# tjcunhao/dpo

Hardware: NVIDIA H100
Metric: rtr_iters_per_sec_sphere2500 (higher is better)
Workload: dtype f64

## Files before the change

dpo_b200/csrc/dpgo_capi.cu:

```cuda
#include <cuda_runtime.h>
#include <algorithm>
#include <chrono>
#include <cmath>
#include <cstdio>
#include <cstdlib>
#include <cstring>
#include <memory>
#include <numeric>
#include <string>
#include <vector>

#include "dpgo_devbuf.cuh"
#include "dpgo_kernels.cuh"

using dpgo::DevBuf;

namespace {

thread_local std::string g_last_error;

int fail(int code, const std::string &msg) {
  g_last_error = msg;
  return code;
}
// ... 275 lines not shown
    DPGO_CUDA(dpgo::launch_pack_sym(D.pinv.get(), (int)N, nchunks, D.sym_segptr.get(), nseg, D.sym_off.get(), D.ppack.get(),
                                    p->stream));
    DPGO_CUDA(cudaStreamSynchronize(p->stream));
    D.sym_ok = 1;
  }
  return DPGO_OK;
}

void nd_fill_info(const dpgo::nd::Hierarchy &H, const dpgo::nd::Plan &P, int64_t *info) {
  for (int i = 0; i < 16; ++i) info[i] = 0;
  int smax = 0, bmax = 0;
  for (const auto &m : H.nodes) { smax = std::max(smax, (int)m.own.size() * H.dh); bmax = std::max(bmax, (int)m.bnd.size() * H.dh); }
  info[0] = H.nstages; info[1] = (int64_t)H.nodes.size(); info[2] = (int64_t)P.phases.size(); info[3] = H.blob_doubles * 8;
  info[4] = P.bytes_per_apply; info[5] = smax; info[6] = bmax; info[7] = H.nd_depth; info[8] = (int64_t)P.steps.size();
  info[9] = (int64_t)P.jobs.size(); info[10] = (int64_t)P.epis.size(); info[11] = P.max_ytiles; info[12] = P.max_slots;
}

dpgo::nd::Options nd_options(int grid, int r, bool cluster = false) {
  dpgo::nd::Options opt;
  opt.grid = grid;
  opt.r = r;
  if (cluster) opt.t_phase_us = 2.0;
  opt.warps = dpgo::OPT_THREADS / 32;
  opt.ycap_tiles = dpgo::ND_YCAP_TILES;
  opt.slot_cap = dpgo::ND_SLOT_CAP;
  if (const char *e = std::getenv("DPGO_ND_CUTS")) opt.force_ncuts = std::atoi(e);
  if (const char *e = std::getenv("DPGO_ND_LEAF")) opt.leaf_size = std::max(1, std::atoi(e));
  if (const char *e = std::getenv("DPGO_ND_TPHASE_US")) opt.t_phase_us = std::atof(e);
  if (const char *e = std::getenv("DPGO_ND_BW_GBS")) opt.bw_gbs = std::atof(e);
  if (const char *e = std::getenv("DPGO_ND_TTILE_US")) opt.t_tile_us = std::atof(e);
// ... 14 lines not shown
  nd::Plan plan;
  std::vector<double> blob;
  auto H = std::make_unique<nd::Hierarchy>();
  try {
    const nd::Options opt = nd_options(p->grid, p->r, p->cluster);
    nd::BsrView Q{p->n, p->dh, p->bsr.h_rowptr.data(), p->bsr.h_bcol.data(), p->bsr.h_bval.data()};
    nd::build_hierarchy(Q, opt, *H);
    nd::build_numeric(Q, opt, *H, blob);
    nd::build_plan(*H, opt, plan);
  } catch (const std::exception &e) {
    return fail(DPGO_ERR_UNSUPPORTED, std::string("sparse exact preconditioner setup: ") + e.what());
  }
  if (plan.max_ytiles > dpgo::ND_YCAP_TILES || plan.max_slots > dpgo::ND_SLOT_CAP)
    return fail(DPGO_ERR_UNSUPPORTED, "sparse exact preconditioner: plan exceeds the shared-memory capacities");
  dpgo_problem::Nd &F = p->nd;
  nd_fill_info(*H, plan, F.info);
  if ((int)plan.phases.size() > dpgo::nd::MAX_PHASES)
    return fail(DPGO_ERR_UNSUPPORTED, "sparse exact preconditioner: too many phases");
  F.H = std::move(H);
  dpgo::KNd &K = F.k;
  for (size_t k = 0; k < plan.phases.size(); ++k) { K.dir[k] = plan.phases[k].dir; K.cta0[k] = plan.phases[k].cta0; }
  K.max_ytiles = std::max(plan.max_ytiles, 1);
  K.max_slots = std::max(plan.max_slots, 1);
  K.max_gathers = K.max_ytiles;
  DPGO_CUDA(F.cta_phase.assign(plan.cta_phase.data(), plan.cta_phase.size(), p->stream));
  DPGO_CUDA(F.steps.assign(plan.steps.data(), plan.steps.size(), p->stream));
  DPGO_CUDA(F.gathers.assign(plan.gathers.data(), plan.gathers.size(), p->stream));
  DPGO_CUDA(F.jobs.assign(plan.jobs.data(), plan.jobs.size(), p->stream));
  DPGO_CUDA(F.epis.assign(plan.epis.data(), plan.epis.size(), p->stream));
  DPGO_CUDA(F.csrc.assign(plan.csrc.data(), plan.csrc.size(), p->stream));
  DPGO_CUDA(F.blob.assign(blob.data(), blob.size(), p->stream));
  K.cta_phase = F.cta_phase.get(); K.steps = F.steps.get(); K.gathers = F.gathers.get(); K.jobs = F.jobs.get();
  K.epis = F.epis.get(); K.csrc = F.csrc.get(); K.blob = F.blob.get();
  const size_t tile = (size_t)p->ts;
  DPGO_CUDA(F.TX.alloc(tile * (size_t)p->n));
  DPGO_CUDA(F.C.alloc(tile * (size_t)F.H->cbuf_tiles));
  K.TX = F.TX.get();
  K.C = F.C.get();
  DPGO_CUDA(cudaMemsetAsync(K.TX, 0, sizeof(double) * tile * (size_t)p->n, p->stream));
// ... 748 lines not shown
  namespace nd = dpgo::nd;
  try {
    nd::Options opt = nd_options(grid, r);
    opt.force_ncuts = force_cuts;
    opt.shift = shift;
    if (leaf_size > 0) opt.leaf_size = leaf_size;
    nd::BsrView Q{n, dh, rowptr.data(), bc.data(), bv.data()};
    nd::Hierarchy H;
    nd::Plan plan;
    std::vector<double> blob;
    nd::build_hierarchy(Q, opt, H);
    nd::build_numeric(Q, opt, H, blob);
    nd::build_plan(H, opt, plan);
    if (plan.max_ytiles > opt.ycap_tiles || plan.max_slots > opt.slot_cap)
      return fail(DPGO_ERR_UNSUPPORTED, "plan exceeds the shared-memory capacities");
    nd::emulate_apply(H, plan, blob, r, V_host, Z_host);
    if (info16) nd_fill_info(H, plan, info16);
    if (const char *dump = std::getenv("DPGO_ND_DUMP_PLAN")) {
      if (FILE *fp = std::fopen(dump, "w")) {
        std::fprintf(fp, "phase,dir,stage,cta,steps,gather_tiles,jobs,job_cols,max_warp_cols,epis\n");
        for (size_t ph = 0; ph < plan.phases.size(); ++ph)
          for (int c = 0; c < plan.grid; ++c) {
            const nd::CtaPhase &cp = plan.cta_phase[(size_t)plan.phases[ph].cta0 + c];
            long gt = 0, nj = 0, jc = 0, ne = 0, mw = 0;
            for (int si = cp.s0; si < cp.s1; ++si) {
              const nd::Step &st = plan.steps[(size_t)si];
              gt += st.g1 - st.g0; nj += st.j1 - st.j0; ne += st.e1 - st.e0;
              std::vector<long> w((size_t)opt.warps, 0);
              for (int j = st.j0; j < st.j1; ++j) { jc += plan.jobs[(size_t)j].ncols; w[(size_t)((j - st.j0) % opt.warps)] += plan.jobs[(size_t)j].ncols + 40; }
              mw += *std::max_element(w.begin(), w.end());
            }
            std::fprintf(fp, "%zu,%d,%d,%d,%d,%ld,%ld,%ld,%ld,%ld\n", ph, plan.phases[ph].dir, plan.phases[ph].stage, c, cp.s1 - cp.s0, gt, nj, jc, mw, ne);
          }
        std::fclose(fp);
      }
    }
  } catch (const std::exception &e) {
    return fail(DPGO_ERR_UNSUPPORTED, std::string("sparse exact preconditioner: ") + e.what());
  }
  return DPGO_OK;
}

static int reassemble_Q(dpgo_problem *p) {
  const dpgo_problem::Edges &E = p->edges;
  DPGO_CUDA(dpgo::launch_assemble_Q(p->bsr.nb, E.cptr.get(), E.contrib.get(), E.T.get(), E.om.get(), E.w.get(), E.sblk.get(),
                                    p->bsr.bval.get(), p->stream));
  DPGO_CUDA(cudaMemcpyAsync(p->bsr.h_bval.data(), p->bsr.bval.get(), sizeof(double) * 16 * (size_t)p->bsr.nb,
// ... 1008 lines not shown
```

dpo_b200/csrc/dpgo_kernels.cu:

```cuda
#include "dpgo_device.cuh"
#include "dpgo_kernels.cuh"
#include "dpgo_rotation.cuh"
#include <cooperative_groups.h>
#include <algorithm>

namespace dpgo {

struct BlockCtx {
  double *sm_warp;
  double *sm_out;
  unsigned epoch;
  int parity;
};

template <int NUSED = NRED>
__device__ __forceinline__ void phase_end(const KParams &kp, BlockCtx &bc, double (&acc)[NRED]) {
  const int lane = threadIdx.x & 31, warp = threadIdx.x >> 5, nwarps = blockDim.x >> 5;
#pragma unroll
  for (int q = 0; q < NUSED; ++q) {
    double v = warp_sum(acc[q]);
    if (lane == 0) bc.sm_warp[warp * NRED + q] = v;
  }
  __syncthreads();
  bc.epoch += gridDim.x;
// ... 598 lines not shown
      }
      double ya[3], sym[3];
      const double z = tangent_project_elem<R, DH>(x, t, it.a, it.c, ya, sym);
      if (ld) {
        Zout[idx] = z;
        acc[0] = fma(z, __ldcg(V + idx), acc[0]);
      }
    }
  }
}

__device__ __forceinline__ int4 ld_int4(const void *p) { return __ldg(reinterpret_cast<const int4 *>(p)); }

template <int R, int DH, bool CLOCK>
__device__ void phase_nd(const KParams &kp, int ph, const double *V, int cb, double *Zout, double *ys, double *slots,
                         int4 *grec, double (&acc)[NRED]) {
  constexpr int TS = R * DH;
  constexpr int SG = SubGroup<R>::SG;
  constexpr int SGW = 32 / SG;
  constexpr int SLOT = nd::PANEL_ROWS * R;
  constexpr int NC = nd::INLINE_CONTRIB;
  const KNd &N = kp.nd;
  const int dir = N.dir[ph];
  const int4 ca = ld_int4(N.cta_phase + N.cta0[ph] + blockIdx.x),
             cbq = ld_int4(reinterpret_cast<const int4 *>(N.cta_phase + N.cta0[ph] + blockIdx.x) + 1);
  const int s0 = ca.x, s1 = ca.y;
  const int lane = threadIdx.x & 31, warp = threadIdx.x >> 5, nwarps = blockDim.x >> 5;
  const int sgw = lane / SG, l = lane & (SG - 1), a = l >> 2, c = l & 3;
  const bool valid = (a < R) && (c < DH);
  const int e = c * R + a;
  const int nsub = nwarps * SGW;
// ... 43 lines not shown
      }
    }
    __syncthreads();
    if (ticking) asm volatile("mov.u64 %0, %%globaltimer;" : "=l"(tg1));
    {
      const int r8 = lane >> 2, k4 = lane & 3;
      const bool bval_lane = (r8 < R);
      int ji = j0 + warp;
      int4 ja = make_int4(0, 0, 0, 0), jb = make_int4(0, 0, 0, 0);
      if (ji < j1) { ja = ld_int4(N.jobs + ji); jb = ld_int4(reinterpret_cast<const int4 *>(N.jobs + ji) + 1); }
      while (ji < j1) {
        const int jn = ji + nwarps;
        int4 na = make_int4(0, 0, 0, 0), nb = make_int4(0, 0, 0, 0);
        if (jn < j1) { na = ld_int4(N.jobs + jn); nb = ld_int4(reinterpret_cast<const int4 *>(N.jobs + jn) + 1); }
        const long long mat = ((long long)(unsigned)ja.x) | ((long long)ja.y << 32);
        const int ncols = ja.z, ycol = ja.w, slot = jb.x, accum = jb.y;
        const double *mp = N.blob + mat + (size_t)k4 * nd::PANEL_ROWS + r8;
        const double *yp = ys + (size_t)(ycol + k4) * R + (bval_lane ? r8 : 0);
        double d0 = 0.0, d1 = 0.0, f0 = 0.0, f1 = 0.0;
        for (int j = 0; j < ncols; j += 32) {
          double am[8], bm[8];
          if (j + 32 <= ncols) {
#pragma unroll
            for (int u = 0; u < 8; ++u) am[u] = ld_stream(mp + (size_t)(j + 4 * u) * nd::PANEL_ROWS);
#pragma unroll
            for (int u = 0; u < 8; ++u) bm[u] = bval_lane ? yp[(size_t)(j + 4 * u) * R] : 0.0;
          } else {
#pragma unroll
            for (int u = 0; u < 8; ++u) am[u] = (j + 4 * u + k4 < ncols) ? ld_stream(mp + (size_t)(j + 4 * u) * nd::PANEL_ROWS) : 0.0;
#pragma unroll
            for (int u = 0; u < 8; ++u) bm[u] = (bval_lane && j + 4 * u + k4 < ncols) ? yp[(size_t)(j + 4 * u) * R] : 0.0;
          }
#pragma unroll
          for (int u = 0; u < 8; u += 2) {
            dmma884(d0, d1, am[u], bm[u]);
            dmma884(f0, f1, am[u + 1], bm[u + 1]);
          }
        }
        d0 += f0;
        d1 += f1;
        {
          double *sl = slots + (size_t)slot * SLOT + r8 * R + 2 * k4;
          if (2 * k4 < R) sl[0] = accum ? sl[0] + d0 : d0;
          if (2 * k4 + 1 < R) sl[1] = accum ? sl[1] + d1 : d1;
        }
        ji = jn; ja = na; jb = nb;
// ... 186 lines not shown
  bc.parity = 0;
  unsigned long long tick_last = 0;
  const bool ticking = FULL && (kp.phase_ns != nullptr) && blockIdx.x == 0 && threadIdx.x == 0;
  auto tick = [&](int kind) {
    if (ticking) {
      unsigned long long t;
      asm volatile("mov.u64 %0, %%globaltimer;" : "=l"(t));
      if (kind >= 0) kp.phase_ns[kind] += t - tick_last;
      tick_last = t;
    }
  };
  tick(-1);
  const dpgo_opt_params_t prm = kp.prm;
  const int precond = prm.precond;
  const bool exact = (precond == DPGO_PRECOND_DENSE_EXACT) || (precond == DPGO_PRECOND_SPARSE_EXACT);
  double acc[NRED];
  double *nd_ys = sV;
  double *nd_slots = sV + (size_t)kp.nd.max_ytiles * R * DH;
  int4 *nd_grec = reinterpret_cast<int4 *>((reinterpret_cast<uintptr_t>(nd_slots + (size_t)kp.nd.max_slots * nd::PANEL_ROWS * R) + 15) & ~(uintptr_t)15);
  auto apply_exact = [&](const double *Vv, int cbx, double *Zout) {
    if (!FULL || precond == DPGO_PRECOND_SPARSE_EXACT) {
      zero(acc);
      for (int ph = 0; ph < kp.nd.nphases; ++ph) {
        phase_nd<R, DH, FULL>(kp, ph, Vv, cbx, Zout, nd_ys, nd_slots, nd_grec, acc);
        if (ph + 1 < kp.nd.nphases) { phase_end<0>(kp, bc, acc); tick(8 + min(ph, 15)); }
      }
      phase_end<1>(kp, bc, acc);
      tick(8 + min(kp.nd.nphases - 1, 15));
    } else {
      if (dense_sym) phase_dense_sym<R>(kp, Vv, ring, sV, sMeta);
      else if (dense_tma) phase_dense_tma<R>(kp, Vv, sV, ring);
      else phase_dense<R>(kp, Vv, sV);
      zero(acc); phase_end<0>(kp, bc, acc);
      tick(1);
      zero(acc); phase_pz<R, DH>(kp, cr, cbx, Vv, Zout, sV, acc);
      phase_end<1>(kp, bc, acc);
      tick(2);
    }
  };
  dpgo_opt_result_t res;
  res.success = 0; res.tcg_status = DPGO_TCG_NOT_RUN; res.tcg_iterations = 0; res.outer_iterations = 0;
  res.rejections = 0; res.spmv_passes = 0; res.precond_applies = 0; res.reserved0 = 0;
  res.f_init = res.gradnorm_init = res.f_opt = res.gradnorm_opt = res.relative_change = res.elapsed_ms = 0.0;
  res.quad_init = res.lin_init = 0.0;

  int cur = 0;

  if (kp.op == OP_PHASE_BENCH) {
    for (int i = 0; i < prm.tr_max_inner; ++i) { zero(acc); acc[0] = 1.0; phase_end<1>(kp, bc, acc); }
    if (blockIdx.x == 0 && threadIdx.x == 0) { res.f_init = acc[0]; *kp.result = res; *kp.bar_epoch = bc.epoch; }
    return;
  }
  if (kp.op == OP_PRECON) {
    if (exact) {
      apply_exact(kp.v[V_AUX], 0, kp.v[V_Z]);
    } else {
      constexpr int TS = R * DH;
      RowIter<R> it(cr);
      const bool valid = (it.a < R) && (it.c < DH);
// ... 312 lines not shown
    tra = fma(s, s, tra);
  }
  const double r2 = om[0] * rot + om[D] * tra;
  if (resid) resid[e] = r2;
  if (fixed && fixed[e]) return;
  const double r = sqrt(r2);
  double wt = 1.0;
  if (cost == 1) wt = 1.0 / r;
  else if (cost == 2) wt = (r < param) ? 1.0 : param / r;
  else if (cost == 3) wt = (r < param) ? 1.0 : 0.0;
  else if (cost == 4) { const double s = 1.0 + r2; wt = 1.0 / (s * s); }
  else if (cost == 5) wt = gnc_tls_weight(r2, mu, param);
  w[e] = wt;
}

template <int R, int DH> static size_t optimize_smem_doubles(const KParams &kp, bool max_only) {
  const size_t base = (OPT_THREADS / 32) * NRED + 2 * NRED + SP_CACHE_INTS / 2;
  const size_t dense = (size_t)DENSE_PER_MAX * R + (size_t)DENSE_RING_DOUBLES + 2 * DENSE_NST + (size_t)SYM_META_DOUBLES;
  if (max_only || kp.prm.precond == DPGO_PRECOND_DENSE_EXACT) return base + dense;
  if (kp.prm.precond == DPGO_PRECOND_SPARSE_EXACT)
    return base + (size_t)kp.nd.max_ytiles * R * DH + (size_t)(kp.nd.max_slots + 1) * nd::PANEL_ROWS * R + 4 * (size_t)kp.nd.max_gathers + 8;
  return base + 8;
}

template <int R, int DH> static void *optimize_kernel(bool full) {
  return full ? (void *)k_optimize<R, DH, true> : (void *)k_optimize<R, DH, false>;
}

template <int R, int DH> static cudaError_t launch_optimize_t(const KParams &kp_in, cudaStream_t stream) {
  KParams kp = kp_in;
  const bool full = (kp.phase_ns != nullptr) || (kp.prm.precond == DPGO_PRECOND_DENSE_EXACT);
  const void *kern = optimize_kernel<R, DH>(full);
  const size_t smem_max = optimize_smem_doubles<R, DH>(kp, true) * sizeof(double);
  static_assert((size_t)ND_YCAP_TILES * R * DH + (size_t)(ND_SLOT_CAP + 1) * nd::PANEL_ROWS * R + 4 * (size_t)ND_YCAP_TILES + 8 <=
                    (size_t)DENSE_PER_MAX * R + (size_t)DENSE_RING_DOUBLES + 2 * DENSE_NST + (size_t)SYM_META_DOUBLES,
                "the sparse plan's capacities must fit the kernel's maximum shared memory");
  kp.smem_doubles = (int)optimize_smem_doubles<R, DH>(kp, false);
  const size_t smem = (size_t)kp.smem_doubles * sizeof(double);
  static bool attr_set[2][64] = {};
  int dev = 0;
  cudaGetDevice(&dev);
  if (dev < 0 || dev >= 64 || !attr_set[full][dev]) {
    cudaError_t e = cudaFuncSetAttribute(kern, cudaFuncAttributeMaxDynamicSharedMemorySize, (int)smem_max);
    if (e != cudaSuccess) return e;
    if (dev >= 0 && dev < 64) attr_set[full][dev] = true;
  }
  {
    static int last_pct[2][64];
    static bool init = false;
    if (!init) { for (int i = 0; i < 64; ++i) last_pct[0][i] = last_pct[1][i] = -1; init = true; }
    const int pct = std::min(100, (int)((smem + 2048) * 100 / (228 * 1024)) + 1);
    if (dev >= 0 && dev < 64 && last_pct[full][dev] != pct) {
      cudaFuncSetAttribute(kern, cudaFuncAttributePreferredSharedMemoryCarveout, pct);
      last_pct[full][dev] = pct;
    }
  }
  if (kp.cluster) {
    static bool np_set[2][64] = {};
// ... 10 lines not shown
    cudaLaunchAttribute at[1];
    at[0].id = cudaLaunchAttributeClusterDimension;
    at[0].val.clusterDim.x = (unsigned)kp.grid;
    at[0].val.clusterDim.y = 1;
    at[0].val.clusterDim.z = 1;
    cfg.attrs = at;
    cfg.numAttrs = 1;
    void *args[] = {(void *)&kp};
    return cudaLaunchKernelExC(&cfg, kern, args);
  }
  void *args[] = {(void *)&kp};
  return cudaLaunchCooperativeKernel(kern, dim3(kp.grid), dim3(OPT_THREADS), args, smem, stream);
}

template <int R, int DH> static int max_cluster_t(int device) {
  const size_t smem = ((OPT_THREADS / 32) * NRED + 2 * NRED + SP_CACHE_INTS / 2 + (size_t)ND_SMEM_NEED_SMALL) * sizeof(double);
  for (int f = 0; f < 2; ++f) cudaFuncSetAttribute(optimize_kernel<R, DH>(f != 0), cudaFuncAttributeNonPortableClusterSizeAllowed, 1);
  for (int cs : {16, 8}) {
    cudaLaunchConfig_t cfg = {};
    cfg.gridDim = dim3(cs);
    cfg.blockDim = dim3(OPT_THREADS);
    cfg.dynamicSmemBytes = smem;
    cudaLaunchAttribute at[1];
    at[0].id = cudaLaunchAttributeClusterDimension;
    at[0].val.clusterDim.x = (unsigned)cs;
    at[0].val.clusterDim.y = 1;
    at[0].val.clusterDim.z = 1;
    cfg.attrs = at;
    cfg.numAttrs = 1;
    int n0 = 0, n1 = 0;
    if (cudaOccupancyMaxActiveClusters(&n0, optimize_kernel<R, DH>(false), &cfg) == cudaSuccess && n0 >= 1 &&
        cudaOccupancyMaxActiveClusters(&n1, optimize_kernel<R, DH>(true), &cfg) == cudaSuccess && n1 >= 1)
      return cs;
  }
  cudaGetLastError();
  return 0;
}

template <int R, int DH> static int max_grid_t(int device) {
  const size_t smem = ((OPT_THREADS / 32) * NRED + 2 * NRED + SP_CACHE_INTS / 2 + (size_t)DENSE_PER_MAX * R + (size_t)DENSE_RING_DOUBLES + 2 * DENSE_NST + (size_t)SYM_META_DOUBLES) * sizeof(double);
  int per_sm = 1, sms = 0;
  for (int f = 0; f < 2; ++f) {
    const void *kern = optimize_kernel<R, DH>(f != 0);
    cudaFuncSetAttribute(kern, cudaFuncAttributeMaxDynamicSharedMemorySize, (int)smem);
    int ps = 0;
    if (cudaOccupancyMaxActiveBlocksPerMultiprocessor(&ps, kern, OPT_THREADS, smem) != cudaSuccess) return 0;
    per_sm = std::min(per_sm, ps);
  }
  if (cudaDeviceGetAttribute(&sms, cudaDevAttrMultiProcessorCount, device) != cudaSuccess) return 0;
  return per_sm > 0 ? sms : 0;
}

cudaError_t launch_optimize(int r, int dh, const KParams &kp, cudaStream_t stream) {
  cudaError_t e = cudaErrorInvalidValue;
  DPGO_DISPATCH(r, dh, e = (launch_optimize_t<R, DH>(kp, stream)));
  return e;
// ... 135 lines not shown
```

dpo_b200/csrc/dpgo_kernels.cuh:

```cuda
#pragma once
#include <cuda_runtime.h>
#include <stdint.h>
#include "../../include/dpgo_b200.h"
#include "nd_precond.h"

namespace dpgo {

enum VecId {
  V_X0 = 0, V_X1,
  V_EG0, V_EG1,
  V_RG0, V_RG1,
  V_Z00, V_Z01,
  V_ETA, V_RES, V_Z,
  V_D0, V_D1,
  V_HD,
  V_T,
  V_XIN,
  V_AUX,
  V_COUNT
};

enum OpCode {
  OP_OPTIMIZE = 0,
  OP_EVAL = 1,
  OP_RHESS = 2,
  OP_PRECON = 3,
  OP_RETRACT = 4,
  OP_PHASE_BENCH = 9,
};

constexpr int NRED = 4;
constexpr int OPT_THREADS = 512;
constexpr int SPMV_GROUP_BLOCKS = 192;
constexpr int ND_YCAP_TILES = 600;
constexpr int ND_SLOT_CAP = 240;
constexpr int ND_SMEM_NEED_SMALL = 16000;
constexpr int SP_CACHE_INTS = 2048;
constexpr int DENSE_PER_MAX = 512;

struct KNd {
  int nphases;
  int max_ytiles, max_slots;
  int max_gathers;
  int dir[nd::MAX_PHASES];
  int cta0[nd::MAX_PHASES];
  const nd::CtaPhase *cta_phase;
  const nd::Step *steps;
  const nd::Gather *gathers;
  const nd::Job *jobs;
  const nd::Epi *epis;
  const int *csrc;
  const double *blob;
  double *TX;
  double *C;
};

struct KParams {
  int n;
// ... 48 lines not shown
        case 3: { constexpr int R = 3, DH = 3; __VA_ARGS__; } break;     \
        case 5: { constexpr int R = 5, DH = 3; __VA_ARGS__; } break;     \
        default: break;                                                  \
      }                                                                  \
    }                                                                    \
  } while (0)

cudaError_t launch_optimize(int r, int dh, const KParams &kp, cudaStream_t stream);
cudaError_t launch_spmv(int r, int dh, int n, const int *rowptr, const int *bcol, const double *bval,
                        const double *X, const double *G, double *out, cudaStream_t stream);
cudaError_t launch_spmv_tma(int r, int dh, int ngroups, const int2 *groups, const int *rowptr, const int *bcol,
                            const double *bval, const double *X, const double *G, double *out, int sms,
                            cudaStream_t stream);
int spmv_group_blocks();
int optimize_max_grid(int r, int dh, int device);
int optimize_max_cluster(int r, int dh, int device);
cudaError_t launch_stiefel_project(int r, int dh, int n, const double *M, double *out, cudaStream_t stream, double c0 = 1.0,
                                   const double *B = nullptr, double c1 = 0.0, const double *C = nullptr, double c2 = 0.0);
cudaError_t launch_pack_tiles(int ts, int count, const int *pose, const double *X, double *out, cudaStream_t stream,
                              const unsigned char *gate = nullptr);
cudaError_t launch_build_G(int r, int dh, int nposes, const int *pose_ids, const int *pose_ptr, const int *edge_slot,
                           const int *edge_out, const double *edge_T, const double *edge_om, const double *gathered,
                           double *G, cudaStream_t stream, const unsigned char *gate = nullptr);
cudaError_t launch_assemble_Q(int64_t nb, const int *cptr, const int2 *contrib, const double *eT, const double *eom, const double *ew,
                              const double *sblk, double *bval, cudaStream_t stream);
cudaError_t launch_edge_weights(int r, int dh, int64_t m, const int *p1, const int *p2, const double *eT, const double *eom,
                                const int *fixed, const double *X, int cost, double mu, double param, double *w, double *resid,
                                cudaStream_t stream);
cudaError_t launch_pack_sym(const double *pinv, int N, int nchunks, const int *segptr, int nseg, const long long *off, double *ppack,
                            cudaStream_t stream);
// ... 65 lines not shown
```

dpo_b200/csrc/nd_precond.cpp:

```cpp
#include "nd_precond.h"

#include <algorithm>
#include <cmath>
#include <cstdio>
#include <cstring>
#include <functional>
#include <numeric>
#include <sstream>
#include <stdexcept>

namespace dpgo {
namespace nd {

namespace {

struct Graph {
  int n = 0;
  std::vector<int> ptr, adj;
};

Graph make_graph(const BsrView &Q) {
  Graph g;
  g.n = Q.n;
  std::vector<std::vector<int>> nb((size_t)Q.n);
// ... 820 lines not shown
  P.grid = opt.grid;
  P.r = opt.r;
  PhaseBuilder pb(H, opt, P);
  for (int st = 0; st < H.nstages; ++st) {
    pb.dir = 0;
    pb.stage = st;
    pb.build();
  }
  for (int st = H.nstages - 2; st >= 0; --st) {
    pb.dir = 1;
    pb.stage = st;
    pb.build();
  }
}

void emulate_apply(const Hierarchy &H, const Plan &P, const std::vector<double> &blob, int r, const double *V, double *Z) {
  const int dh = H.dh, ts = r * dh;
  std::vector<double> TX((size_t)H.n * ts, 0.0), C((size_t)H.cbuf_tiles * ts, 0.0);
  std::vector<double> ys((size_t)std::max(P.max_ytiles, 1) * ts), slots((size_t)std::max(P.max_slots, 1) * PANEL_ROWS * r);
  for (size_t ph = 0; ph < P.phases.size(); ++ph) {
    const Phase &phs = P.phases[ph];
    for (int c = 0; c < P.grid; ++c) {
      const CtaPhase &cph = P.cta_phase[(size_t)phs.cta0 + c];
      const int s0 = cph.s0, s1 = cph.s1;
      if (s1 > s0) {
        const Step &f = P.steps[(size_t)s0];
        if (f.g0 != cph.g0 || f.g1 != cph.g1 || f.j0 != cph.j0 || f.j1 != cph.j1 || f.e0 != cph.e0 || f.e1 != cph.e1)
          throw std::runtime_error("nd: inline first step disagrees with the step table");
      }
      std::fill(slots.begin(), slots.end(), std::nan(""));
      for (int si = s0; si < s1; ++si) {
// ... 2 lines not shown
        for (int gi = st.g0; gi < st.g1; ++gi) {
          const Gather &g = P.gathers[(size_t)gi];
          for (int e = 0; e < ts; ++e) {
            double v = (phs.dir == 0) ? V[(size_t)g.src * ts + e] : TX[(size_t)g.src * ts + e];
            for (int k = 0; k < g.nc; ++k) {
              const int ct = (k < INLINE_CONTRIB) ? g.ci[k] : P.csrc[(size_t)(g.cext + k - INLINE_CONTRIB)];
              v -= C[(size_t)ct * ts + e];
            }
            ys[(size_t)g.ytile * ts + e] = v;
          }
        }
        for (int ji = st.j0; ji < st.j1; ++ji) {
          const Job &jb = P.jobs[(size_t)ji];
          const double *mat = blob.data() + jb.mat;
          double *sl = slots.data() + (size_t)jb.slot * PANEL_ROWS * r;
          for (int row = 0; row < PANEL_ROWS; ++row)
            for (int a = 0; a < r; ++a) {
              double acc = 0.0;
              for (int j = 0; j < jb.ncols; ++j) acc += mat[(size_t)j * PANEL_ROWS + row] * ys[(size_t)(jb.ycol + j) * r + a];
              if (jb.accum) sl[row * r + a] += acc; else sl[row * r + a] = acc;
            }
        }
        for (int ei = st.e0; ei < st.e1; ++ei) {
          const Epi &ep = P.epis[(size_t)ei];
          for (int cc = 0; cc < dh; ++cc)
            for (int a = 0; a < r; ++a) {
              const int e = cc * r + a, row = ep.half * dh + cc;
              double sum = 0.0;
              for (int k = 0; k < ep.nslots; ++k) sum += slots[(size_t)(ep.slot0 + k) * PANEL_ROWS * r + row * r + a];
              if (ep.kind == EPI_F_OWN) {
                TX[(size_t)ep.out * ts + e] = sum;
              } else if (ep.kind == EPI_F_BND) {
                for (int k = 0; k < ep.nc; ++k) {
                  const int ct = (k < INLINE_CONTRIB) ? ep.ci[k] : P.csrc[(size_t)(ep.cext + k - INLINE_CONTRIB)];
// ... 9 lines not shown
                Z[(size_t)ep.aux * ts + e] = x;
              }
            }
        }
      }
    }
  }
}

std::string describe(const Hierarchy &H, const Plan &P) {
  std::ostringstream os;
  os << "nd: n=" << H.n << " depth=" << H.nd_depth << " cuts=[";
  for (size_t k = 0; k < H.cuts.size(); ++k) os << (k ? "," : "") << H.cuts[k];
  os << "] stages=" << H.nstages << " nodes=" << H.nodes.size() << " blob=" << (H.blob_doubles * 8) / 1e6 << "MB phases=" << P.phases.size()
     << " bytes/apply=" << P.bytes_per_apply / 1e6 << "MB steps=" << P.steps.size() << " jobs=" << P.jobs.size() << " epis=" << P.epis.size()
     << " max_ytiles=" << P.max_ytiles << " max_slots=" << P.max_slots;
  for (int st = 0; st < H.nstages; ++st) {
    int cnt = 0, smax = 0, bmax = 0;
    for (const MacroNode &m : H.nodes)
      if (m.stage == st) { ++cnt; smax = std::max(smax, (int)m.own.size()); bmax = std::max(bmax, (int)m.bnd.size()); }
    os << " | stage " << st << ": " << cnt << " nodes, own<=" << smax << " bnd<=" << bmax;
  }
  return os.str();
}

}
}
```

dpo_b200/csrc/nd_precond.h:

```cpp
#pragma once
#include <cstdint>
#include <string>
#include <vector>

namespace dpgo {
namespace nd {

struct Step { int g0, g1, j0, j1, e0, e1, pad0, pad1; };
struct CtaPhase { int s0, s1; int g0, g1, j0, j1, e0, e1; };
constexpr int INLINE_CONTRIB = 4;
struct Gather { int ytile; int src; int nc; int cext; int ci[INLINE_CONTRIB]; };
struct Job { long long mat; int ncols; int ycol; int slot; int accum; int pad0, pad1; };
struct Epi { int kind; int slot0; int nslots; int half; int out; int aux; int nc; int cext; int ci[INLINE_CONTRIB]; };
enum EpiKind { EPI_F_OWN = 0, EPI_F_BND = 1, EPI_B_OWN = 2, EPI_ROOT = 3 };
struct Phase { int dir; int stage; int cta0; int pad; };
constexpr int MAX_PHASES = 16;

constexpr int PANEL_ROWS = 8;

struct Options {
  int grid = 132;
  int r = 5;
  int warps = 16;
  int leaf_size = 12;
  int max_cuts = 3;
  int ycap_tiles = 600;
  int slot_cap = 240;
  double t_phase_us = 3.5;
  double t_tile_us = 0.012;
  double bw_gbs = 3000.0;
  int force_ncuts = -1;
  double shift = 0.1;
};
// ... 21 lines not shown
  std::vector<int> cuts;
  int nd_depth = 0;
};

struct Plan {
  std::vector<Phase> phases;
  std::vector<CtaPhase> cta_phase;
  std::vector<Step> steps;
  std::vector<Gather> gathers;
  std::vector<Job> jobs;
  std::vector<Epi> epis;
  std::vector<int> csrc;
  int grid = 0, r = 0;
  int max_ytiles = 0, max_slots = 0;
  int64_t bytes_per_apply = 0;
};

struct BsrView { int n; int dh; const int *rowptr; const int *bcol; const double *bval; };

void build_hierarchy(const BsrView &Q, const Options &opt, Hierarchy &H);
struct DenseNodeOps {
  virtual bool factor(int s, int b, double *Foo, double *Fob, double *Fbb) = 0;
  virtual ~DenseNodeOps() {}
};
void build_numeric(const BsrView &Q, const Options &opt, Hierarchy &H, std::vector<double> &blob, DenseNodeOps *big_node = nullptr,
                   int big_threshold = 1 << 30);
void build_plan(const Hierarchy &H, const Options &opt, Plan &P);
void emulate_apply(const Hierarchy &H, const Plan &P, const std::vector<double> &blob, int r, const double *V, double *Z);

std::string describe(const Hierarchy &H, const Plan &P);

}
}
```

dpo_b200/problem.py:

```python
from __future__ import annotations

import ctypes as C
from typing import Optional

import numpy as np

from . import _capi as capi
from ._capi import (ALG_RGD, ALG_RTR, PRECOND_BLOCK_JACOBI, PRECOND_DENSE_EXACT, PRECOND_NONE, PRECOND_SPARSE_EXACT,
                    OptParams, OptResult)


class ROPTALG:
    RTR = ALG_RTR
    RGD = ALG_RGD


class QuadraticProblem:

    def __init__(self, n: int, d: int, r: int, device: int = 0,
                 preconditioners=(PRECOND_BLOCK_JACOBI, PRECOND_SPARSE_EXACT), cluster: bool = False):
        self._lib = capi.load_library()
        self.n, self.d, self.r = int(n), int(d), int(r)
        self.N = (self.d + 1) * self.n
        self.device = device
# ... 215 lines not shown
        return p.value

    def spmv_device(self, x_ptr: int, out_ptr: int, add_G: bool = False) -> None:
        capi.check(self._lib.dpgo_spmv_device(self._h, C.c_void_p(x_ptr), C.c_void_p(out_ptr), int(add_G)))

    def spmv_algorithmic_bytes(self, add_G: bool = False) -> int:
        return int(self._lib.dpgo_spmv_algorithmic_bytes(self._h, int(add_G)))

    def nd_ready(self) -> bool:
        return bool(self._precond_mask & (1 << PRECOND_SPARSE_EXACT))

    def nd_info(self) -> dict:
        info = (C.c_int64 * 16)()
        capi.check(self._lib.dpgo_nd_info(self._h, info))
        keys = ("levels", "nodes", "phases", "block_bytes", "bytes_per_apply", "max_own", "max_bnd", "nd_depth", "steps",
                "jobs", "epilogues", "max_ytiles", "max_slots")
        return {k: int(info[i]) for i, k in enumerate(keys)}

    def precond_algorithmic_bytes(self, preconditioner: int) -> int:
        return int(self._lib.dpgo_precond_algorithmic_bytes(self._h, int(preconditioner)))

    def resident_f_gradnorm(self):
        fo, nrm = C.c_double(), C.c_double()
        capi.check(self._lib.dpgo_agent_f_rgradnorm_resident(self._h, C.byref(fo), C.byref(nrm)))
        return fo.value, nrm.value


class QuadraticOptimizer:

    def __init__(self, problem: QuadraticProblem):
        self.problem = problem
        self._lib = problem._lib
# ... 67 lines not shown
```

Before: 1932.

## Keep part of sparse preconditioner factor panels resident in shared memory across applies

Adds a planner that greedily assigns leading columns of each warp's factor-panel jobs to a per-CTA shared-memory resident region, using the shared memory left over under a fixed limit. On the first preconditioner apply the kernel streams panels from global memory and also copies them into shared memory. Later applies read those columns from shared memory, which cuts global/L2 traffic for the triangular solves. In exchange the kernel always requests the maximum dynamic shared memory, and the host emulator gains a fill pass.

```diff
diff --git a/dpo_b200/csrc/dpgo_capi.cu b/dpo_b200/csrc/dpgo_capi.cu
--- a/dpo_b200/csrc/dpgo_capi.cu
+++ b/dpo_b200/csrc/dpgo_capi.cu
@@ -313,6 +313,14 @@
   info[0] = H.nstages; info[1] = (int64_t)H.nodes.size(); info[2] = (int64_t)P.phases.size(); info[3] = H.blob_doubles * 8;
   info[4] = P.bytes_per_apply; info[5] = smax; info[6] = bmax; info[7] = H.nd_depth; info[8] = (int64_t)P.steps.size();
   info[9] = (int64_t)P.jobs.size(); info[10] = (int64_t)P.epis.size(); info[11] = P.max_ytiles; info[12] = P.max_slots;
+  info[13] = P.resident_bytes; info[14] = (int64_t)P.max_resident_doubles * 8;
+}
+
+void nd_kernel_sizes(const dpgo::nd::Plan &plan, dpgo::KNd &K) {
+  K.max_ytiles = std::max(plan.max_ytiles, 1);
+  K.max_slots = std::max(plan.max_slots, 1);
+  K.max_gathers = K.max_ytiles;
+  K.resident_doubles = 0;
 }
 
 dpgo::nd::Options nd_options(int grid, int r, bool cluster = false) {
@@ -357,15 +365,19 @@
   if (plan.max_ytiles > dpgo::ND_YCAP_TILES || plan.max_slots > dpgo::ND_SLOT_CAP)
     return fail(DPGO_ERR_UNSUPPORTED, "sparse exact preconditioner: plan exceeds the shared-memory capacities");
   dpgo_problem::Nd &F = p->nd;
-  nd_fill_info(*H, plan, F.info);
   if ((int)plan.phases.size() > dpgo::nd::MAX_PHASES)
     return fail(DPGO_ERR_UNSUPPORTED, "sparse exact preconditioner: too many phases");
+  dpgo::KNd &K = F.k;
+  nd_kernel_sizes(plan, K);
+  try {
+    nd::assign_residency(plan, dpgo::OPT_THREADS / 32, p->cluster ? 0 : dpgo::nd_resident_budget(p->r, p->dh, K));
+  } catch (const std::exception &e) {
+    return fail(DPGO_ERR_UNSUPPORTED, std::string("sparse exact preconditioner setup: ") + e.what());
+  }
+  K.resident_doubles = plan.max_resident_doubles;
+  nd_fill_info(*H, plan, F.info);
   F.H = std::move(H);
-  dpgo::KNd &K = F.k;
   for (size_t k = 0; k < plan.phases.size(); ++k) { K.dir[k] = plan.phases[k].dir; K.cta0[k] = plan.phases[k].cta0; }
-  K.max_ytiles = std::max(plan.max_ytiles, 1);
-  K.max_slots = std::max(plan.max_slots, 1);
-  K.max_gathers = K.max_ytiles;
   DPGO_CUDA(F.cta_phase.assign(plan.cta_phase.data(), plan.cta_phase.size(), p->stream));
   DPGO_CUDA(F.steps.assign(plan.steps.data(), plan.steps.size(), p->stream));
   DPGO_CUDA(F.gathers.assign(plan.gathers.data(), plan.gathers.size(), p->stream));
@@ -1144,6 +1156,11 @@
     nd::build_plan(H, opt, plan);
     if (plan.max_ytiles > opt.ycap_tiles || plan.max_slots > opt.slot_cap)
       return fail(DPGO_ERR_UNSUPPORTED, "plan exceeds the shared-memory capacities");
+    dpgo::KNd K = {};
+    nd_kernel_sizes(plan, K);
+    int64_t budget = dpgo::nd_resident_budget(r, dh, K);
+    if (const char *e = std::getenv("DPGO_ND_RESIDENT_BYTES")) budget = std::atoll(e);
+    nd::assign_residency(plan, opt.warps, budget);
     nd::emulate_apply(H, plan, blob, r, V_host, Z_host);
     if (info16) nd_fill_info(H, plan, info16);
     if (const char *dump = std::getenv("DPGO_ND_DUMP_PLAN")) {
@@ -1161,6 +1178,22 @@
               mw += *std::max_element(w.begin(), w.end());
             }
             std::fprintf(fp, "%zu,%d,%d,%d,%d,%ld,%ld,%ld,%ld,%ld\n", ph, plan.phases[ph].dir, plan.phases[ph].stage, c, cp.s1 - cp.s0, gt, nj, jc, mw, ne);
+          }
+        std::fclose(fp);
+      }
+    }
+    if (const char *dump = std::getenv("DPGO_ND_DUMP_JOBS")) {
+      if (FILE *fp = std::fopen(dump, "w")) {
+        std::fprintf(fp, "phase,cta,step,warp,ncols,nres,soff,budget\n");
+        for (size_t ph = 0; ph < plan.phases.size(); ++ph)
+          for (int c = 0; c < plan.grid; ++c) {
+            const nd::CtaPhase &cp = plan.cta_phase[(size_t)plan.phases[ph].cta0 + c];
+            for (int si = cp.s0; si < cp.s1; ++si)
+              for (int j = plan.steps[(size_t)si].j0; j < plan.steps[(size_t)si].j1; ++j) {
+                const nd::Job &jb = plan.jobs[(size_t)j];
+                std::fprintf(fp, "%zu,%d,%d,%d,%d,%d,%d,%lld\n", ph, c, si, (j - plan.steps[(size_t)si].j0) % opt.warps, jb.ncols,
+                             jb.nres, jb.soff, (long long)budget);
+              }
           }
         std::fclose(fp);
       }
diff --git a/dpo_b200/csrc/dpgo_kernels.cu b/dpo_b200/csrc/dpgo_kernels.cu
--- a/dpo_b200/csrc/dpgo_kernels.cu
+++ b/dpo_b200/csrc/dpgo_kernels.cu
@@ -636,7 +636,7 @@
 
 template <int R, int DH, bool CLOCK>
 __device__ void phase_nd(const KParams &kp, int ph, const double *V, int cb, double *Zout, double *ys, double *slots,
-                         int4 *grec, double (&acc)[NRED]) {
+                         int4 *grec, double *sres, bool fill, double (&acc)[NRED]) {
   constexpr int TS = R * DH;
   constexpr int SG = SubGroup<R>::SG;
   constexpr int SGW = 32 / SG;
@@ -710,13 +710,20 @@
         int4 na = make_int4(0, 0, 0, 0), nb = make_int4(0, 0, 0, 0);
         if (jn < j1) { na = ld_int4(N.jobs + jn); nb = ld_int4(reinterpret_cast<const int4 *>(N.jobs + jn) + 1); }
         const long long mat = ((long long)(unsigned)ja.x) | ((long long)ja.y << 32);
-        const int ncols = ja.z, ycol = ja.w, slot = jb.x, accum = jb.y;
+        const int ncols = ja.z, ycol = ja.w, slot = jb.x, accum = jb.y, nres = jb.w;
         const double *mp = N.blob + mat + (size_t)k4 * nd::PANEL_ROWS + r8;
         const double *yp = ys + (size_t)(ycol + k4) * R + (bval_lane ? r8 : 0);
+        double *rp = sres + jb.z + lane;
         double d0 = 0.0, d1 = 0.0, f0 = 0.0, f1 = 0.0;
         for (int j = 0; j < ncols; j += 32) {
           double am[8], bm[8];
-          if (j + 32 <= ncols) {
+          const bool res = j < nres;
+          if (res && !fill) {
+#pragma unroll
+            for (int u = 0; u < 8; ++u) am[u] = (j + 4 * u < ncols) ? rp[(size_t)(j + 4 * u) * nd::PANEL_ROWS] : 0.0;
+#pragma unroll
+            for (int u = 0; u < 8; ++u) bm[u] = (bval_lane && j + 4 * u + k4 < ncols) ? yp[(size_t)(j + 4 * u) * R] : 0.0;
+          } else if (j + 32 <= ncols) {
 #pragma unroll
             for (int u = 0; u < 8; ++u) am[u] = ld_stream(mp + (size_t)(j + 4 * u) * nd::PANEL_ROWS);
 #pragma unroll
@@ -726,6 +733,11 @@
             for (int u = 0; u < 8; ++u) am[u] = (j + 4 * u + k4 < ncols) ? ld_stream(mp + (size_t)(j + 4 * u) * nd::PANEL_ROWS) : 0.0;
 #pragma unroll
             for (int u = 0; u < 8; ++u) bm[u] = (bval_lane && j + 4 * u + k4 < ncols) ? yp[(size_t)(j + 4 * u) * R] : 0.0;
+          }
+          if (res && fill) {
+#pragma unroll
+            for (int u = 0; u < 8; ++u)
+              if (j + 4 * u < ncols) rp[(size_t)(j + 4 * u) * nd::PANEL_ROWS] = am[u];
           }
 #pragma unroll
           for (int u = 0; u < 8; u += 2) {
@@ -942,15 +954,21 @@
   const dpgo_opt_params_t prm = kp.prm;
   const int precond = prm.precond;
   const bool exact = (precond == DPGO_PRECOND_DENSE_EXACT) || (precond == DPGO_PRECOND_SPARSE_EXACT);
+  dpgo_opt_result_t res;
+  res.success = 0; res.tcg_status = DPGO_TCG_NOT_RUN; res.tcg_iterations = 0; res.outer_iterations = 0;
+  res.rejections = 0; res.spmv_passes = 0; res.precond_applies = 0; res.reserved0 = 0;
+  res.f_init = res.gradnorm_init = res.f_opt = res.gradnorm_opt = res.relative_change = res.elapsed_ms = 0.0;
+  res.quad_init = res.lin_init = 0.0;
   double acc[NRED];
   double *nd_ys = sV;
   double *nd_slots = sV + (size_t)kp.nd.max_ytiles * R * DH;
   int4 *nd_grec = reinterpret_cast<int4 *>((reinterpret_cast<uintptr_t>(nd_slots + (size_t)kp.nd.max_slots * nd::PANEL_ROWS * R) + 15) & ~(uintptr_t)15);
+  double *nd_res = reinterpret_cast<double *>(nd_grec + 2 * (size_t)kp.nd.max_gathers);
   auto apply_exact = [&](const double *Vv, int cbx, double *Zout) {
     if (!FULL || precond == DPGO_PRECOND_SPARSE_EXACT) {
       zero(acc);
       for (int ph = 0; ph < kp.nd.nphases; ++ph) {
-        phase_nd<R, DH, FULL>(kp, ph, Vv, cbx, Zout, nd_ys, nd_slots, nd_grec, acc);
+        phase_nd<R, DH, FULL>(kp, ph, Vv, cbx, Zout, nd_ys, nd_slots, nd_grec, nd_res, res.precond_applies == 0, acc);
         if (ph + 1 < kp.nd.nphases) { phase_end<0>(kp, bc, acc); tick(8 + min(ph, 15)); }
       }
       phase_end<1>(kp, bc, acc);
@@ -966,11 +984,6 @@
       tick(2);
     }
   };
-  dpgo_opt_result_t res;
-  res.success = 0; res.tcg_status = DPGO_TCG_NOT_RUN; res.tcg_iterations = 0; res.outer_iterations = 0;
-  res.rejections = 0; res.spmv_passes = 0; res.precond_applies = 0; res.reserved0 = 0;
-  res.f_init = res.gradnorm_init = res.f_opt = res.gradnorm_opt = res.relative_change = res.elapsed_ms = 0.0;
-  res.quad_init = res.lin_init = 0.0;
 
   int cur = 0;
 
@@ -1313,13 +1326,23 @@
   w[e] = wt;
 }
 
-template <int R, int DH> static size_t optimize_smem_doubles(const KParams &kp, bool max_only) {
+template <int R, int DH> static size_t nd_staged_doubles(const KNd &nd) {
+  return (OPT_THREADS / 32) * NRED + 2 * NRED + SP_CACHE_INTS / 2 + (size_t)nd.max_ytiles * R * DH +
+         (size_t)(nd.max_slots + 1) * nd::PANEL_ROWS * R + 4 * (size_t)nd.max_gathers + 8;
+}
+
+template <int R, int DH> static size_t optimize_smem_doubles(const KParams &kp) {
   const size_t base = (OPT_THREADS / 32) * NRED + 2 * NRED + SP_CACHE_INTS / 2;
   const size_t dense = (size_t)DENSE_PER_MAX * R + (size_t)DENSE_RING_DOUBLES + 2 * DENSE_NST + (size_t)SYM_META_DOUBLES;
-  if (max_only || kp.prm.precond == DPGO_PRECOND_DENSE_EXACT) return base + dense;
-  if (kp.prm.precond == DPGO_PRECOND_SPARSE_EXACT)
-    return base + (size_t)kp.nd.max_ytiles * R * DH + (size_t)(kp.nd.max_slots + 1) * nd::PANEL_ROWS * R + 4 * (size_t)kp.nd.max_gathers + 8;
+  if (kp.prm.precond == DPGO_PRECOND_DENSE_EXACT) return base + dense;
+  if (kp.prm.precond == DPGO_PRECOND_SPARSE_EXACT) return nd_staged_doubles<R, DH>(kp.nd) + (size_t)kp.nd.resident_doubles;
   return base + 8;
+}
+
+int64_t nd_resident_budget(int r, int dh, const KNd &nd) {
+  int64_t staged = 0;
+  DPGO_DISPATCH(r, dh, staged = (int64_t)nd_staged_doubles<R, DH>(nd) * (int64_t)sizeof(double));
+  return std::max<int64_t>(0, (int64_t)OPT_SMEM_LIMIT - staged);
 }
 
 template <int R, int DH> static void *optimize_kernel(bool full) {
@@ -1330,17 +1353,16 @@
   KParams kp = kp_in;
   const bool full = (kp.phase_ns != nullptr) || (kp.prm.precond == DPGO_PRECOND_DENSE_EXACT);
   const void *kern = optimize_kernel<R, DH>(full);
-  const size_t smem_max = optimize_smem_doubles<R, DH>(kp, true) * sizeof(double);
   static_assert((size_t)ND_YCAP_TILES * R * DH + (size_t)(ND_SLOT_CAP + 1) * nd::PANEL_ROWS * R + 4 * (size_t)ND_YCAP_TILES + 8 <=
                     (size_t)DENSE_PER_MAX * R + (size_t)DENSE_RING_DOUBLES + 2 * DENSE_NST + (size_t)SYM_META_DOUBLES,
                 "the sparse plan's capacities must fit the kernel's maximum shared memory");
-  kp.smem_doubles = (int)optimize_smem_doubles<R, DH>(kp, false);
+  kp.smem_doubles = (int)optimize_smem_doubles<R, DH>(kp);
   const size_t smem = (size_t)kp.smem_doubles * sizeof(double);
   static bool attr_set[2][64] = {};
   int dev = 0;
   cudaGetDevice(&dev);
   if (dev < 0 || dev >= 64 || !attr_set[full][dev]) {
-    cudaError_t e = cudaFuncSetAttribute(kern, cudaFuncAttributeMaxDynamicSharedMemorySize, (int)smem_max);
+    cudaError_t e = cudaFuncSetAttribute(kern, cudaFuncAttributeMaxDynamicSharedMemorySize, OPT_SMEM_LIMIT);
     if (e != cudaSuccess) return e;
     if (dev >= 0 && dev < 64) attr_set[full][dev] = true;
   }
@@ -1381,8 +1403,11 @@
 }
 
 template <int R, int DH> static int max_cluster_t(int device) {
-  const size_t smem = ((OPT_THREADS / 32) * NRED + 2 * NRED + SP_CACHE_INTS / 2 + (size_t)ND_SMEM_NEED_SMALL) * sizeof(double);
-  for (int f = 0; f < 2; ++f) cudaFuncSetAttribute(optimize_kernel<R, DH>(f != 0), cudaFuncAttributeNonPortableClusterSizeAllowed, 1);
+  const size_t smem = OPT_SMEM_LIMIT;
+  for (int f = 0; f < 2; ++f) {
+    cudaFuncSetAttribute(optimize_kernel<R, DH>(f != 0), cudaFuncAttributeNonPortableClusterSizeAllowed, 1);
+    cudaFuncSetAttribute(optimize_kernel<R, DH>(f != 0), cudaFuncAttributeMaxDynamicSharedMemorySize, OPT_SMEM_LIMIT);
+  }
   for (int cs : {16, 8}) {
     cudaLaunchConfig_t cfg = {};
     cfg.gridDim = dim3(cs);
@@ -1405,8 +1430,10 @@
 }
 
 template <int R, int DH> static int max_grid_t(int device) {
-  const size_t smem = ((OPT_THREADS / 32) * NRED + 2 * NRED + SP_CACHE_INTS / 2 + (size_t)DENSE_PER_MAX * R + (size_t)DENSE_RING_DOUBLES + 2 * DENSE_NST + (size_t)SYM_META_DOUBLES) * sizeof(double);
-  int per_sm = 1, sms = 0;
+  const size_t smem = OPT_SMEM_LIMIT;
+  int per_sm = 1, sms = 0, optin = 0;
+  if (cudaDeviceGetAttribute(&optin, cudaDevAttrMaxSharedMemoryPerBlockOptin, device) != cudaSuccess || optin < OPT_SMEM_LIMIT)
+    return 0;
   for (int f = 0; f < 2; ++f) {
     const void *kern = optimize_kernel<R, DH>(f != 0);
     cudaFuncSetAttribute(kern, cudaFuncAttributeMaxDynamicSharedMemorySize, (int)smem);
diff --git a/dpo_b200/csrc/dpgo_kernels.cuh b/dpo_b200/csrc/dpgo_kernels.cuh
--- a/dpo_b200/csrc/dpgo_kernels.cuh
+++ b/dpo_b200/csrc/dpgo_kernels.cuh
@@ -34,7 +34,7 @@
 constexpr int SPMV_GROUP_BLOCKS = 192;
 constexpr int ND_YCAP_TILES = 600;
 constexpr int ND_SLOT_CAP = 240;
-constexpr int ND_SMEM_NEED_SMALL = 16000;
+constexpr int OPT_SMEM_LIMIT = 227 * 1024;
 constexpr int SP_CACHE_INTS = 2048;
 constexpr int DENSE_PER_MAX = 512;
 
@@ -42,6 +42,7 @@
   int nphases;
   int max_ytiles, max_slots;
   int max_gathers;
+  int resident_doubles;
   int dir[nd::MAX_PHASES];
   int cta0[nd::MAX_PHASES];
   const nd::CtaPhase *cta_phase;
@@ -120,6 +121,7 @@
                             cudaStream_t stream);
 int spmv_group_blocks();
 int optimize_max_grid(int r, int dh, int device);
+int64_t nd_resident_budget(int r, int dh, const KNd &nd);
 int optimize_max_cluster(int r, int dh, int device);
 cudaError_t launch_stiefel_project(int r, int dh, int n, const double *M, double *out, cudaStream_t stream, double c0 = 1.0,
                                    const double *B = nullptr, double c1 = 0.0, const double *C = nullptr, double c2 = 0.0);
diff --git a/dpo_b200/csrc/nd_precond.cpp b/dpo_b200/csrc/nd_precond.cpp
--- a/dpo_b200/csrc/nd_precond.cpp
+++ b/dpo_b200/csrc/nd_precond.cpp
@@ -858,7 +858,104 @@
   }
 }
 
+void assign_residency(Plan &P, int warps, int64_t budget_bytes) {
+  const int G = P.grid;
+  for (Job &j : P.jobs) { j.soff = 0; j.nres = 0; }
+  P.resident_doubles.assign((size_t)G, 0);
+  P.max_resident_doubles = 0;
+  P.resident_bytes = 0;
+  const int64_t budget = std::max<int64_t>(0, budget_bytes / 8);
+  const int nph = (int)P.phases.size();
+  auto nrounds = [](int ncols) { return (ncols + RES_ROUND - 1) / RES_ROUND; };
+  for (int c = 0; c < G; ++c) {
+    std::vector<std::vector<std::vector<int>>> seq((size_t)nph);
+    std::vector<std::vector<int>> seq_step((size_t)nph);
+    std::vector<int> level((size_t)nph, 0);
+    for (int ph = 0; ph < nph; ++ph) {
+      const CtaPhase &cp = P.cta_phase[(size_t)P.phases[(size_t)ph].cta0 + c];
+      for (int si = cp.s0; si < cp.s1; ++si) {
+        const Step &st = P.steps[(size_t)si];
+        for (int w = 0; w < warps && st.j0 + w < st.j1; ++w) {
+          std::vector<int> rd;
+          for (int ji = st.j0 + w; ji < st.j1; ji += warps) {
+            const int nc = P.jobs[(size_t)ji].ncols;
+            for (int k = 0; k < nrounds(nc); ++k)
+              rd.push_back(resident_doubles(std::min(nc, (k + 1) * RES_ROUND)) - resident_doubles(k * RES_ROUND));
+          }
+          level[(size_t)ph] = std::max(level[(size_t)ph], (int)rd.size());
+          seq[(size_t)ph].push_back(std::move(rd));
+          seq_step[(size_t)ph].push_back(si);
+        }
+      }
+    }
+    int64_t used = 0;
+    while (true) {
+      int best = -1;
+      int64_t best_cost = 0;
+      double best_score = 0.0;
+      for (int ph = 0; ph < nph; ++ph) {
+        const int L = level[(size_t)ph];
+        if (L == 0) continue;
+        int64_t cost = 0;
+        std::vector<int> steps_hit;
+        for (size_t q = 0; q < seq[(size_t)ph].size(); ++q) {
+          const std::vector<int> &rd = seq[(size_t)ph][q];
+          if ((int)rd.size() < L) continue;
+          cost += rd[rd.size() - (size_t)L];
+          steps_hit.push_back(seq_step[(size_t)ph][q]);
+        }
+        if (used + cost > budget) continue;
+        std::sort(steps_hit.begin(), steps_hit.end());
+        const double saved = (double)(std::unique(steps_hit.begin(), steps_hit.end()) - steps_hit.begin());
+        const double score = (double)cost / saved;
+        if (best < 0 || score < best_score) { best = ph; best_cost = cost; best_score = score; }
+      }
+      if (best < 0) break;
+      --level[(size_t)best];
+      used += best_cost;
+    }
+    int off = 0;
+    for (int ph = 0; ph < nph; ++ph) {
+      const CtaPhase &cp = P.cta_phase[(size_t)P.phases[(size_t)ph].cta0 + c];
+      for (int si = cp.s0; si < cp.s1; ++si) {
+        const Step &st = P.steps[(size_t)si];
+        for (int w = 0; w < warps && st.j0 + w < st.j1; ++w) {
+          int total = 0;
+          for (int ji = st.j0 + w; ji < st.j1; ji += warps) total += nrounds(P.jobs[(size_t)ji].ncols);
+          int left = std::max(0, total - level[(size_t)ph]);
+          for (int ji = st.j0 + w; ji < st.j1 && left > 0; ji += warps) {
+            Job &jb = P.jobs[(size_t)ji];
+            const int take = std::min(left, nrounds(jb.ncols));
+            left -= take;
+            jb.nres = std::min(jb.ncols, take * RES_ROUND);
+            jb.soff = off;
+            off += resident_doubles(jb.nres);
+            P.resident_bytes += (int64_t)jb.nres * PANEL_ROWS * 8;
+          }
+        }
+      }
+    }
+    if (off > budget) throw std::runtime_error("nd: resident region exceeds its budget");
+    P.resident_doubles[(size_t)c] = off;
+    P.max_resident_doubles = std::max(P.max_resident_doubles, off);
+  }
+}
+
+static void emulate_pass(const Hierarchy &H, const Plan &P, const std::vector<double> &blob, int r, const double *V, double *Z,
+                         std::vector<std::vector<double>> &region, bool fill);
+
 void emulate_apply(const Hierarchy &H, const Plan &P, const std::vector<double> &blob, int r, const double *V, double *Z) {
+  const bool resident = P.resident_bytes > 0;
+  std::vector<std::vector<double>> region((size_t)P.grid);
+  for (int c = 0; c < P.grid && resident; ++c) region[(size_t)c].assign((size_t)P.resident_doubles[(size_t)c], std::nan(""));
+  std::vector<double> Zfill;
+  if (resident) Zfill.assign((size_t)r * H.dh * H.n, 0.0);
+  for (int pass = resident ? 0 : 1; pass < 2; ++pass)
+    emulate_pass(H, P, blob, r, V, pass == 0 ? Zfill.data() : Z, region, resident && pass == 0);
+}
+
+static void emulate_pass(const Hierarchy &H, const Plan &P, const std::vector<double> &blob, int r, const double *V, double *Z,
+                         std::vector<std::vector<double>> &region, bool fill) {
   const int dh = H.dh, ts = r * dh;
   std::vector<double> TX((size_t)H.n * ts, 0.0), C((size_t)H.cbuf_tiles * ts, 0.0);
   std::vector<double> ys((size_t)std::max(P.max_ytiles, 1) * ts), slots((size_t)std::max(P.max_slots, 1) * PANEL_ROWS * r);
@@ -891,10 +988,19 @@
           const Job &jb = P.jobs[(size_t)ji];
           const double *mat = blob.data() + jb.mat;
           double *sl = slots.data() + (size_t)jb.slot * PANEL_ROWS * r;
+          auto rslot = [&](int j, int row) -> double & {
+            return region[(size_t)c].at((size_t)jb.soff + (size_t)(j / 4) * 32 + (size_t)(row * 4 + (j & 3)));
+          };
+          if (fill)
+            for (int j = 0; j < jb.nres; ++j)
+              for (int row = 0; row < PANEL_ROWS; ++row) rslot(j, row) = mat[(size_t)j * PANEL_ROWS + row];
           for (int row = 0; row < PANEL_ROWS; ++row)
             for (int a = 0; a < r; ++a) {
               double acc = 0.0;
-              for (int j = 0; j < jb.ncols; ++j) acc += mat[(size_t)j * PANEL_ROWS + row] * ys[(size_t)(jb.ycol + j) * r + a];
+              for (int j = 0; j < jb.ncols; ++j) {
+                const double m = (j < jb.nres && !fill) ? rslot(j, row) : mat[(size_t)j * PANEL_ROWS + row];
+                acc += m * ys[(size_t)(jb.ycol + j) * r + a];
+              }
               if (jb.accum) sl[row * r + a] += acc; else sl[row * r + a] = acc;
             }
         }
@@ -934,7 +1040,9 @@
   for (size_t k = 0; k < H.cuts.size(); ++k) os << (k ? "," : "") << H.cuts[k];
   os << "] stages=" << H.nstages << " nodes=" << H.nodes.size() << " blob=" << (H.blob_doubles * 8) / 1e6 << "MB phases=" << P.phases.size()
      << " bytes/apply=" << P.bytes_per_apply / 1e6 << "MB steps=" << P.steps.size() << " jobs=" << P.jobs.size() << " epis=" << P.epis.size()
-     << " max_ytiles=" << P.max_ytiles << " max_slots=" << P.max_slots;
+     << " max_ytiles=" << P.max_ytiles << " max_slots=" << P.max_slots
+     << " resident=" << (P.bytes_per_apply > 0 ? (double)P.resident_bytes / (double)P.bytes_per_apply : 0.0)
+     << " max_resident_KB=" << P.max_resident_doubles * 8 / 1024.0;
   for (int st = 0; st < H.nstages; ++st) {
     int cnt = 0, smax = 0, bmax = 0;
     for (const MacroNode &m : H.nodes)
diff --git a/dpo_b200/csrc/nd_precond.h b/dpo_b200/csrc/nd_precond.h
--- a/dpo_b200/csrc/nd_precond.h
+++ b/dpo_b200/csrc/nd_precond.h
@@ -10,13 +10,15 @@
 struct CtaPhase { int s0, s1; int g0, g1, j0, j1, e0, e1; };
 constexpr int INLINE_CONTRIB = 4;
 struct Gather { int ytile; int src; int nc; int cext; int ci[INLINE_CONTRIB]; };
-struct Job { long long mat; int ncols; int ycol; int slot; int accum; int pad0, pad1; };
+struct Job { long long mat; int ncols; int ycol; int slot; int accum; int soff, nres; };
 struct Epi { int kind; int slot0; int nslots; int half; int out; int aux; int nc; int cext; int ci[INLINE_CONTRIB]; };
 enum EpiKind { EPI_F_OWN = 0, EPI_F_BND = 1, EPI_B_OWN = 2, EPI_ROOT = 3 };
 struct Phase { int dir; int stage; int cta0; int pad; };
 constexpr int MAX_PHASES = 16;
 
 constexpr int PANEL_ROWS = 8;
+constexpr int RES_ROUND = 32;
+inline int resident_doubles(int nres) { return (nres + 3) / 4 * 32; }
 
 struct Options {
   int grid = 132;
@@ -68,6 +70,9 @@
   int grid = 0, r = 0;
   int max_ytiles = 0, max_slots = 0;
   int64_t bytes_per_apply = 0;
+  std::vector<int> resident_doubles;
+  int max_resident_doubles = 0;
+  int64_t resident_bytes = 0;
 };
 
 struct BsrView { int n; int dh; const int *rowptr; const int *bcol; const double *bval; };
@@ -80,6 +85,7 @@
 void build_numeric(const BsrView &Q, const Options &opt, Hierarchy &H, std::vector<double> &blob, DenseNodeOps *big_node = nullptr,
                    int big_threshold = 1 << 30);
 void build_plan(const Hierarchy &H, const Options &opt, Plan &P);
+void assign_residency(Plan &P, int warps, int64_t budget_bytes);
 void emulate_apply(const Hierarchy &H, const Plan &P, const std::vector<double> &blob, int r, const double *V, double *Z);
 
 std::string describe(const Hierarchy &H, const Plan &P);
diff --git a/dpo_b200/problem.py b/dpo_b200/problem.py
--- a/dpo_b200/problem.py
+++ b/dpo_b200/problem.py
@@ -253,8 +253,10 @@
         info = (C.c_int64 * 16)()
         capi.check(self._lib.dpgo_nd_info(self._h, info))
         keys = ("levels", "nodes", "phases", "block_bytes", "bytes_per_apply", "max_own", "max_bnd", "nd_depth", "steps",
-                "jobs", "epilogues", "max_ytiles", "max_slots")
-        return {k: int(info[i]) for i, k in enumerate(keys)}
+                "jobs", "epilogues", "max_ytiles", "max_slots", "resident_bytes", "max_resident_bytes_per_cta")
+        out = {k: int(info[i]) for i, k in enumerate(keys)}
+        out["resident_fraction"] = out["resident_bytes"] / max(out["bytes_per_apply"], 1)
+        return out
 
     def precond_algorithmic_bytes(self, preconditioner: int) -> int:
         return int(self._lib.dpgo_precond_algorithmic_bytes(self._h, int(preconditioner)))
```

New measurement: 2034 (median of 6 runs). 1.05x the previous value.
